# choderalab/pymbar

Measured on AMD Instinct MI355X. Metric: mbar_adaptive_iterations_per_sec, higher is better.
Workload: dtype f64

## Files before the change

### pymbar_amd/csrc/mbar_capi.cpp

```cpp
#include "mbar_ctx.h"

using namespace mbar;
using namespace mbar::host;

namespace mbar {
namespace host {

int fail(mbar_ctx* c, int code, const std::string& msg) {
    if (c) c->error = msg;
    g_last_error = msg;
    return code;
}
hipEvent_t get_event(mbar_ctx* c) {
    if (!c->pool.empty()) {
        hipEvent_t e = c->pool.back();
        c->pool.pop_back();
        return e;
    }
    hipEvent_t e;
    if (hipEventCreate(&e) != hipSuccess) return nullptr;
    return e;
}
void flush_timers(mbar_ctx* c) {
    for (auto& tp : c->pending) {
// ... 611 lines not shown
    *out = c;
    return MBAR_OK;
}

void mbar_ctx_destroy(mbar_ctx* c) {
    if (!c) return;
    (void)hipSetDevice(c->device);
    if (c->stream) (void)hipStreamSynchronize(c->stream);
    flush_timers(c);
    for (auto e : c->pool) (void)hipEventDestroy(e);
    if (c->comm && g_rccl.CommDestroy) g_rccl.CommDestroy(c->comm);
    if (c->u_alloc) (void)cache_free(c->u_alloc);
    else if (c->u) (void)cache_free(c->u);
    if (c->logden[0]) (void)cache_free(c->logden[0]);
    if (c->ad) (void)cache_free(c->ad);
    if (c->P) (void)cache_free(c->P);
    if (c->pm_vec) (void)cache_free(c->pm_vec);
    if (c->pm_ld0) (void)cache_free(c->pm_ld0);
    if (c->part_g) (void)cache_free(c->part_g);
    if (c->cwsq) (void)cache_free(c->cwsq);
    if (c->chol) (void)cache_free(c->chol);
    if (c->ad_ints) (void)cache_free(c->ad_ints);
    if (c->h_ctl) (void)cache_host_free(c->h_ctl);
    if (c->ad_graph) (void)hipGraphExecDestroy(c->ad_graph);
    if (c->dn) (void)cache_free(c->dn);
    if (c->cw) (void)cache_free(c->cw);
    if (c->lden_eff) (void)cache_free(c->lden_eff);
    if (c->small) (void)cache_free(c->small);
    if (c->part) (void)cache_free(c->part);
    if (c->scratch) (void)cache_free(c->scratch);
    if (c->red) (void)cache_free(c->red);
    if (c->hred) (void)cache_host_free(c->hred);
    if (c->lognum_part) (void)cache_free(c->lognum_part);
    if (c->f_hist) (void)cache_free(c->f_hist);
    if (c->hstage) (void)cache_host_free(c->hstage);
    if (c->vec_tmp) (void)cache_free(c->vec_tmp);
    if (c->boot_idx) (void)cache_free(c->boot_idx);
    if (c->stamps) (void)hipFree(c->stamps);
    if (c->sci_graph) (void)hipGraphExecDestroy(c->sci_graph);
    if (c->stream) {
        std::lock_guard<std::mutex> lock(g_dev_mu);
        auto& pool = g_stream_pool[c->device];
        if (pool.size() < 8)
            pool.push_back(c->stream);
        else
            (void)hipStreamDestroy(c->stream);
// ... 208 lines not shown
    if (!c->vec_tmp) HIPCHK(c, cache_malloc((void**)&c->vec_tmp, (size_t)c->ld * sizeof(double)));
    int* dlabel = nullptr;
    HIPCHK(c, cache_malloc((void**)&dlabel, (size_t)c->N * sizeof(int)));
    c->vec_holds_logshift = false;
    hipError_t e = hipMemcpyAsync(c->vec_tmp, v_host, (size_t)c->N * sizeof(double), hipMemcpyHostToDevice, c->stream);
    if (e == hipSuccess) e = hipMemcpyAsync(dlabel, label_host, (size_t)c->N * sizeof(int), hipMemcpyHostToDevice, c->stream);
    if (e == hipSuccess) e = launch_fill_masked_rows(c->stream, c->u + row0 * c->ld, c->ld, c->N, nrows, c->vec_tmp, dlabel);
    if (e == hipSuccess) e = hipStreamSynchronize(c->stream);
    (void)cache_free(dlabel);
    if (e != hipSuccess) return fail(c, MBAR_ERR_HIP, std::string("mbar_ctx_fill_masked_rows: ") + hipGetErrorString(e));
    c->u_checked = false;
    c->P_valid = false;
    c->last_psum.clear();
    flush_timers(c);
    return MBAR_OK;
}

int mbar_ctx_download_u(mbar_ctx* c, double* out, int64_t ld_out) {
    if (!c || !out || ld_out < c->N) return fail(c, MBAR_ERR_ARG, "bad argument");
    HIPCHK(c, hipSetDevice(c->device));
    const double* src = c->u;
    if (c->opt_debug_download_p) {
        if (!c->P || !c->P_valid) return fail(c, MBAR_ERR_STATE, "no resident probability matrix on this context");
        src = c->P;
    }
    HIPCHK(c, hipMemcpy2DAsync(out, (size_t)ld_out * sizeof(double), src, (size_t)c->ld * sizeof(double),
                               (size_t)c->N * sizeof(double), (size_t)c->K, hipMemcpyDeviceToHost, c->stream));
    return sync_stream(c);
}

int mbar_ctx_generate_harmonic(mbar_ctx* c, uint64_t seed, const double* O_k, const double* K_k,
                               const int64_t* N_k_global, int64_t n_global0) {
    if (!c || !O_k || !K_k || !N_k_global) return fail(c, MBAR_ERR_ARG, "NULL argument");
    HIPCHK(c, hipSetDevice(c->device));
    std::vector<int64_t> cum((size_t)c->K + 1, 0);
    for (int64_t k = 0; k < c->K; ++k) cum[k + 1] = cum[k] + N_k_global[k];
    if (n_global0 < 0 || n_global0 + c->N > cum[c->K]) return fail(c, MBAR_ERR_ARG, "shard exceeds sum(N_k)");
    double* dO = d_misc(c);
    double* dK = d_misc(c) + c->Kp;
    int64_t* dC = reinterpret_cast<int64_t*>(d_misc(c) + 2 * c->Kp);
    HIPCHK(c, hipMemcpyAsync(dO, O_k, c->K * sizeof(double), hipMemcpyHostToDevice, c->stream));
    HIPCHK(c, hipMemcpyAsync(dK, K_k, c->K * sizeof(double), hipMemcpyHostToDevice, c->stream));
    HIPCHK(c, hipMemcpyAsync(dC, cum.data(), (c->K + 1) * sizeof(int64_t), hipMemcpyHostToDevice, c->stream));
    {
        ScopedTimer t(c, MBAR_TIMER_OTHER);
        HIPCHK(c, launch_generate_harmonic(c->stream, c->u, c->ld, c->N, c->K, seed, dO, dK, dC, n_global0));
    }
// ... 706 lines not shown
```

### pymbar_amd/csrc/mbar_ctx.h

```cpp
#pragma once
#include "../../include/mbar_hip.h"
#include "mbar_internal.h"

#include <dlfcn.h>
#include <sched.h>
#include <unistd.h>
#include <rccl/rccl.h>

#include <algorithm>
#include <chrono>
#include <condition_variable>
#include <cmath>
#include <cstdio>
#include <cstdlib>
#include <cstring>
#include <functional>
#include <limits>
#include <map>
#include <memory>
#include <mutex>
#include <string>
#include <atomic>
#include <thread>
#include <unordered_map>
// ... 229 lines not shown
    double* scratch = nullptr;
    size_t scratch_doubles = 0;
    double* red = nullptr;
    size_t red_doubles = 0;
    double* hred = nullptr;
    double* hstage = nullptr;
    double* lognum_part = nullptr;
    size_t lognum_part_doubles = 0;
    double* f_hist = nullptr;
    double* vec_tmp = nullptr;
    int64_t* boot_idx = nullptr;
    size_t boot_idx_words = 0;
    uint64_t boot_layout_digest[2] = {0, 0};
    int64_t boot_states = 0, boot_total = 0;
    bool boot_has_order = false;
    bool vec_holds_logshift = false;
    hipGraphExec_t sci_graph = nullptr;
    int64_t sci_graph_batch = 0, sci_graph_sig = 0;
    double sci_graph_tol = 0.0;
    double* ad = nullptr;
    int64_t ad_hist_cap = 0;
    int* ad_ints = nullptr;
    int* h_ctl = nullptr;
    hipGraphExec_t ad_graph = nullptr;
    int64_t ad_graph_batch = 0, ad_graph_sig = 0;
    double* P = nullptr;
    bool P_failed = false;
    double* pm_vec = nullptr;
    double* pm_ld0 = nullptr;
    double* part_g = nullptr;
    size_t part_g_doubles = 0;
    double* cwsq = nullptr;
    double* chol = nullptr;
    long long* stamps = nullptr;
    std::vector<double> last_psum;
    bool P_valid = false;
    std::vector<double> P_a0;
    int64_t opt_grid = 0, opt_force_generic = 0, opt_check_finite = 1, opt_sci_batch = 16, opt_timing = 0, opt_graph = 1, opt_small = 1, opt_wide = 1;
    int64_t opt_device_loop = 1, opt_adapt_batch = 8, opt_pmode = 1, opt_fused = 1, opt_quad = 1, opt_device_loop_wide = 1, opt_pcache = 1, opt_merge_select = 1, opt_sci_merged = 1, opt_wide_pmode = 1, opt_quad_trim = 1, opt_light_last = 1, opt_direct_results = 1, opt_debug_download_p = 0, opt_fused_general = 0;
    int64_t opt_small_balanced = 1, opt_sci_pingpong = 1, opt_host_pmode = 2, opt_rect_waves = 8, opt_newton_ldlt = 1;

    ncclComm_t comm = nullptr;
    mbar_loopback* loop = nullptr;
    mbar_allreduce_fn host_reduce = nullptr;
    void* host_reduce_user = nullptr;
    int rank = 0, nranks = 1;
// ... 220 lines not shown
```

### pymbar_amd/csrc/mbar_internal.h

```cpp
#pragma once
#include <hip/hip_runtime.h>
#include <stdint.h>

#include "../../include/mbar_hip.h"

namespace mbar {

constexpr int TS = 16;
constexpr int GROUPS = 4;
constexpr int MAX_FAST_K = 256;
constexpr int PANEL = 64;

inline int64_t padded_K(int64_t K) {
    if (K <= 128) return (K + 15) / 16 * 16;
    return (K + PANEL - 1) / PANEL * PANEL;
}
inline int lse_nb_for(int64_t Kp) {
    static const int nbs[] = {1, 2, 3, 4, 5, 6, 7, 8, 12, 16};
    int need = (int)(Kp / 16);
    for (int nb : nbs) if (nb >= need) return nb;
    return 0;
}

#if defined(__HIPCC__)
// ... 164 lines not shown
    int64_t hist_cap;
    int pmode;
    const double* a0;
    double* ccur;
    int fused;
    double* cgram;
    int light_ok;
    long long* stamps;
    int newton_ldlt;
};
LaunchGeom psweep_geometry(int nb, int num_cu, int64_t ntiles, int64_t grid_override);
hipError_t launch_psweep(hipStream_t s, int nb, int nf, const LaunchGeom& g, const double* P, int64_t ld, int64_t N,
                         const double* cmul, const double* cw, double* rinv0, double* rinv1, double* psum_part,
                         const LoopCtl& lc = LoopCtl());
LaunchGeom fused_geometry(int nb, int num_cu, int64_t ntiles, int64_t grid_override, bool unit = false);
hipError_t launch_fused(hipStream_t s, int nb, const LaunchGeom& g, const double* P, int64_t ld, int64_t N, const double* cmul,
                        const double* cw, const double* wsq, bool unit, double* rinv_base, double* gram_part, double* psum_part,
                        const LoopCtl& lc);
LaunchGeom build_sweep_geometry(int nb, int num_cu, int64_t ntiles, int64_t grid_override);
hipError_t launch_build_sweep(hipStream_t s, int nb, const LaunchGeom& g, const double* u, int64_t ld, int64_t N,
                              const double* aden, const double* cw, double* P, double* rinv_slot, double* psum_part);
LaunchGeom build_gram_geometry(int nb, int num_cu, int64_t ntiles, int64_t grid_override);
hipError_t launch_build_gram(hipStream_t s, int nb, const LaunchGeom& g, const double* u, int64_t ld, int64_t N,
                             const double* aden, const double* wsq, bool general, double* P, double* rinv_slot, double* gram_part);

hipError_t launch_make_p(hipStream_t s, int num_cu, const double* u, int64_t ld, int64_t N, int64_t rows, const double* aden,
                         const double* logden, double* P);
hipError_t launch_fill(hipStream_t s, double* v, double value, int64_t n);
hipError_t launch_zero(hipStream_t s, void* p, size_t bytes);
hipError_t launch_sqrt_vec(hipStream_t s, double* dst, const double* src, int64_t n);
hipError_t launch_rinv_from_logden(hipStream_t s, const double* ld0, const double* ldv, const double* cw, bool weighted, int64_t N,
                                   double* out);
hipError_t launch_rinv_weighted(hipStream_t s, const double* rinv, const double* cw, int64_t N, double* out,
                                const LoopCtl& lc = LoopCtl());
hipError_t launch_newton(hipStream_t s, const AdaptArgs& a);
constexpr size_t NEWTON_CHOL_WORK = (size_t)256 * 256 + 8;
hipError_t launch_newton_chol(hipStream_t s, const AdaptArgs& a, double* work);
hipError_t launch_select(hipStream_t s, const AdaptArgs& a);
hipError_t launch_select_newton(hipStream_t s, const AdaptArgs& a);
hipError_t launch_ctl_resume(hipStream_t s, int* ctl);


enum : int { KDE_GAUSSIAN = 0, KDE_TOPHAT = 1, KDE_EPANECHNIKOV = 2, KDE_EXPONENTIAL = 3, KDE_LINEAR = 4, KDE_COSINE = 5 };
constexpr int KDE_MAX_D = 8;
constexpr int KDE_TILE = 64;
constexpr int KDE_MAX_CB = 32;
struct KdeLaunch {
    int kernel, d, cb;
    const double* X;
    int64_t ldx;
    const double* V;
    const double* Q;
    int64_t ldq, M;
    double coef;
    double h, inv_h, inv_h2;
    int64_t qblocks, nchunks, chunk;
    double* part;
};
size_t kde_lds_bytes(int kernel, int d, int cb);
hipError_t launch_kde(hipStream_t s, const KdeLaunch& a);
hipError_t launch_kde_combine(hipStream_t s, const KdeLaunch& a, int cv, const double* logW, double lognorm, double* out, int* flag);
hipError_t launch_kde_exact(hipStream_t s, const KdeLaunch& a, int64_t N, int64_t npairs, const int64_t* pq, const double* logW,
                            double lognorm, double* out);
// ... 418 lines not shown
```

### pymbar_amd/csrc/mbar_k_pmode.hip

```cpp
#include "mbar_device.h"

namespace mbar {

__global__ void __launch_bounds__(256)
k_rinv_weighted(const double* __restrict__ rinv, const double* __restrict__ cw, int64_t N, double* __restrict__ out,
                const int* __restrict__ ctl, int64_t slot_stride) {
    if (ctl) {
        if (ctl[CTL_DONE] != 0) return;
        rinv += (int64_t)ctl[CTL_SLOT] * slot_stride;
    }
    for (int64_t n = (int64_t)blockIdx.x * blockDim.x + threadIdx.x; n < N; n += (int64_t)gridDim.x * blockDim.x)
        out[n] = rinv[n] * sqrt(cw[n]);
}

__global__ void __launch_bounds__(256)
k_rinv_from_logden(const double* __restrict__ ld0, const double* __restrict__ ldv, const double* __restrict__ cw, int weighted,
                   int64_t N, double* __restrict__ out) {
    for (int64_t n = (int64_t)blockIdx.x * blockDim.x + threadIdx.x; n < N; n += (int64_t)gridDim.x * blockDim.x) {
        double r = exp(ld0[n] - ldv[n]);
        if (weighted) r *= sqrt(cw[n]);
        out[n] = r;
    }
}
hipError_t launch_rinv_from_logden(hipStream_t s, const double* ld0, const double* ldv, const double* cw, bool weighted, int64_t N,
// ... 502 lines not shown
    return stage_offsets_wide(ld) ? go(k_build_sweep<NB, true>) : go(k_build_sweep<NB, false>);
}
LaunchGeom build_sweep_geometry(int nb, int num_cu, int64_t ntiles, int64_t grid_override) {
    return lse_geometry(nb, 1, num_cu, ntiles, grid_override, 1);
}
hipError_t launch_build_sweep(hipStream_t s, int nb, const LaunchGeom& g, const double* u, int64_t ld, int64_t N,
                              const double* aden, const double* cw, double* P, double* rinv_slot, double* pp) {
    switch (nb) {
#define MBAR_CASE(NB_) \
    case NB_: return launch_build_sweep_nb<NB_>(s, g, u, ld, N, aden, cw, P, rinv_slot, pp);
        MBAR_CASE(1) MBAR_CASE(2) MBAR_CASE(3) MBAR_CASE(4) MBAR_CASE(5) MBAR_CASE(6) MBAR_CASE(7) MBAR_CASE(8)
#undef MBAR_CASE
        default: return hipErrorInvalidValue;
    }
}

LaunchGeom build_gram_geometry(int nb, int num_cu, int64_t ntiles, int64_t grid_override) {
    LaunchGeom g = fused_geometry(nb, num_cu, ntiles, grid_override);
    g.lds_bytes = (size_t)4 * 2 * ((size_t)nb * 16 * TS * 8 + TS * 8) + EXP_TABLE_BYTES;
    return g;
}
template <int NB>
static hipError_t launch_build_gram_nb(hipStream_t s, const LaunchGeom& g, const double* u, int64_t ld, int64_t N,
                                       const double* aden, const double* wsq, bool general, double* P, double* rinv_slot, double* gp) {
    auto go = [&](auto kern) -> hipError_t {
        if (g.lds_bytes > 64 * 1024) {
            hipError_t e = hipFuncSetAttribute(reinterpret_cast<const void*>(kern),
                                               hipFuncAttributeMaxDynamicSharedMemorySize, (int)g.lds_bytes);
            if (e != hipSuccess) return e;
        }
        const int64_t ntiles = (N + TS - 1) / TS;
        hipLaunchKernelGGL(kern, dim3(g.blocks), dim3(256), g.lds_bytes, s, u, ld, N, ntiles, aden, wsq, P, rinv_slot, gp);
        return hipGetLastError();
    };
    if (general) return stage_offsets_wide(ld) ? go(k_build_gram<NB, true, true>) : go(k_build_gram<NB, false, true>);
    return stage_offsets_wide(ld) ? go(k_build_gram<NB, true, false>) : go(k_build_gram<NB, false, false>);
}
hipError_t launch_build_gram(hipStream_t s, int nb, const LaunchGeom& g, const double* u, int64_t ld, int64_t N,
                             const double* aden, const double* wsq, bool general, double* P, double* rinv_slot, double* gram_part) {
    switch (nb) {
#define MBAR_CASE(NB_) \
    case NB_: return launch_build_gram_nb<NB_>(s, g, u, ld, N, aden, wsq, general, P, rinv_slot, gram_part);
        MBAR_CASE(1) MBAR_CASE(2) MBAR_CASE(3) MBAR_CASE(4) MBAR_CASE(5) MBAR_CASE(6) MBAR_CASE(7) MBAR_CASE(8)
#undef MBAR_CASE
        default: return hipErrorInvalidValue;
    }
}

}
```

### pymbar_amd/csrc/mbar_k_solver.hip

```cpp
#include "mbar_device.h"

namespace mbar {

__global__ void __launch_bounds__(256)
k_reduce(const double* __restrict__ part, int64_t nparts, int64_t count, int64_t chunk,
         double* __restrict__ out) {
    const int64_t i = (int64_t)blockIdx.x * blockDim.x + threadIdx.x;
    if (i >= count) return;
    const int64_t p0 = (int64_t)blockIdx.y * chunk;
    const int64_t p1 = p0 + chunk < nparts ? p0 + chunk : nparts;
    double s = 0.0;
#pragma unroll 8
    for (int64_t p = p0; p < p1; ++p) s += part[p * count + i];
    out[(int64_t)blockIdx.y * count + i] = s;
}

constexpr int LN_ROWS = 8;
constexpr int LN_TILE = 64;
template <bool MASKED>
__device__ __forceinline__ void lognum_tile(const double* __restrict__ u, int64_t ld, int64_t N, int64_t K, int64_t k0,
                                            int64_t n, const double* __restrict__ logden, const double (&a)[LN_ROWS],
                                            double (&m)[LN_ROWS], double (&s)[LN_ROWS]) {
    const bool ok = !MASKED || n < N;
    const int64_t nn = ok ? n : 0;
// ... 1188 lines not shown
    select_body(q, gram_in_lds ? select_dyn_lds : nullptr, st);
    __syncthreads();
    if (st && threadIdx.x == 0) st[1] = clock64();
    newton_body_ldlt<NB>(q, select_dyn_lds, gram_in_lds ? select_dyn_lds : nullptr, st);
    if (st && threadIdx.x == 0) st[5] = clock64();
}

__global__ void __launch_bounds__(256)
k_loop_reduce(LoopSrc src, int64_t count, int op, double* __restrict__ out) {
    const int64_t i = (int64_t)blockIdx.x * blockDim.x + threadIdx.x;
    if (i >= count) return;
    double v = src.p[0][i];
    for (int r = 1; r < src.n; ++r) v = op == 0 ? v + src.p[r][i] : fmax(v, src.p[r][i]);
    out[i] = v;
}

__global__ void k_ctl_resume(int* ctl) {
    if (threadIdx.x == 0 && ctl[CTL_DONE] == 3) {
        ctl[CTL_DONE] = 0;
        ctl[CTL_NEEDGRAM] = 0;
    }
}



hipError_t launch_reduce(hipStream_t s, const double* part, int64_t nparts, int64_t count, double* scratch,
                         double* out) {
    const unsigned gx = (unsigned)((count + 255) / 256);
    if (nparts <= 32) {
        hipLaunchKernelGGL(k_reduce, dim3(gx, 1), dim3(256), 0, s, part, nparts, count, nparts, out);
        return hipGetLastError();
    }
    const int64_t chunk = 32;
    const int64_t n1 = (nparts + chunk - 1) / chunk;
    hipLaunchKernelGGL(k_reduce, dim3(gx, (unsigned)n1), dim3(256), 0, s, part, nparts, count, chunk, scratch);
    hipLaunchKernelGGL(k_reduce, dim3(gx, 1), dim3(256), 0, s, (const double*)scratch, n1, count, n1, out);
    return hipGetLastError();
}

static int64_t lognum_tiles_per_chunk(int64_t N, int64_t K) {
    const int64_t ntiles = (N + LN_TILE - 1) / LN_TILE;
    const int64_t nsb = (K + LN_ROWS - 1) / LN_ROWS;
    int64_t target = 16384 / nsb;
    if (target < 1) target = 1;
    int64_t tpc = (ntiles + target - 1) / target;
    return tpc < 1 ? 1 : tpc;
// ... 237 lines not shown
    if (count < 1 || src.n < 1 || src.n > 8) return hipErrorInvalidValue;
    hipLaunchKernelGGL(k_loop_reduce, dim3((unsigned)((count + 255) / 256)), dim3(256), 0, s, src, count, op, out);
    return hipGetLastError();
}

hipError_t launch_newton_chol(hipStream_t s, const AdaptArgs& a, double* work) {
    const int M = a.m - 1;
    if (M < 0 || M > CHOL_NP - 1 || a.Kp > 256) return hipErrorInvalidValue;
    double* Aw = work;
    double* thr = work + (size_t)CHOL_NP * CHOL_NP;
    hipLaunchKernelGGL(k_chol_setup, dim3(CHOL_NP / 16, CHOL_NP / 16), dim3(256), 0, s, a, Aw, thr);
    for (int j0 = 0; j0 < M; j0 += CB) {
        hipLaunchKernelGGL(k_chol_panel, dim3(1), dim3(256), 0, s, a, Aw, (const double*)thr, j0);
        const int rows_below = M + 1 - (j0 + CB);
        if (rows_below > 0) {
            const int nt = (rows_below + CB - 1) / CB;
            hipLaunchKernelGGL(k_chol_update, dim3((unsigned)(nt * (nt + 1) / 2)), dim3(256), 0, s, a, Aw, j0);
        }
    }
    hipLaunchKernelGGL(k_chol_finish, dim3(1), dim3(256), 0, s, a, (const double*)Aw);
    return hipGetLastError();
}

hipError_t launch_ctl_resume(hipStream_t s, int* ctl) {
    hipLaunchKernelGGL(k_ctl_resume, dim3(1), dim3(64), 0, s, ctl);
    return hipGetLastError();
}

hipError_t launch_select_newton(hipStream_t s, const AdaptArgs& a) {
    const int M = a.m - 1;
    if (M > 127 || a.Kp > 128) return hipErrorInvalidValue;
    const int stage = (a.fused && a.Kp == 128) ? 1 : 0;
    const size_t lds = a.newton_ldlt ? (size_t)LDLT_LDS_DOUBLES * sizeof(double) : stage ? (size_t)SELECT_GRAM_LDS_DOUBLES * sizeof(double) : 0;
    auto go = [&](auto kern) -> hipError_t {
        if (lds > 48 * 1024) {
            hipError_t e = hipFuncSetAttribute(reinterpret_cast<const void*>(kern), hipFuncAttributeMaxDynamicSharedMemorySize, (int)lds);
            if (e != hipSuccess) return e;
        }
        hipLaunchKernelGGL(kern, dim3(1), dim3(256), lds, s, a, stage);
        return hipGetLastError();
    };
    if (a.newton_ldlt) return a.Kp <= 64 ? go(k_select_newton_ldlt<4>) : go(k_select_newton_ldlt<8>);
    if (M <= 63) return go(k_select_newton<4>);
    return go(k_select_newton<8>);
}

// ... 81 lines not shown
```

### pymbar_amd/csrc/mbar_loops.cpp

```cpp
#include "mbar_ctx.h"

using namespace mbar;
using namespace mbar::host;

namespace mbar {
namespace host {

int adaptive_host_loop(mbar_ctx* c, std::vector<double>& f, double tol, int64_t maxiter, int64_t min_sc_iter, double gamma,
                       int check_convergence, double* history, int64_t history_rows, mbar_solve_result& res,
                       std::vector<double>& psum, double& max_delta) {
    const int64_t K = c->K;
    const int m = (int)c->sampled.size();
    const int first = c->sampled[0];
    std::vector<double> f_old(K), cand(2 * (size_t)K), psum2(2 * (size_t)K);
    std::vector<double> H((size_t)m * m), g(m), x;
    std::vector<int> pos((size_t)K, -1);
    for (int i = 0; i < m; ++i) pos[(size_t)c->sampled[i]] = i;
    psum.assign(K, 0.0);
    int cur = 0;
    int rc = eval_core(c, f.data(), 1, 0, c->logden[cur], nullptr, psum.data(), nullptr, nullptr);
    if (rc) return rc;
    bool done = false;
    const GramPlan plan = plan_for(c);
    const bool dbg = std::getenv("MBAR_DEBUG_TIMING") != nullptr;
// ... 225 lines not shown
    const int64_t nit = res.iterations - it0;
    if (dbg && nit > 0)
        std::fprintf(stderr, "[mbar] adaptive (host loop): %lld it, per it: passA %.3f ms (of it unpacking %.3f), host solve %.3f ms (of it the factorisation + substitutions %.3f), passB %.3f ms, total %.3f ms\n",
                     (long long)nit, tA / nit, tA_unpack / nit, tH / nit, tH_solve / nit, tB / nit, (now_ms() - t0) / nit);
    return MBAR_OK;
}

bool device_loop_eligible(const mbar_ctx* c) {
    if (!c->opt_device_loop || !use_fast(c)) return false;
    if (c->nranks > 1 && !stream_transport(c)) return false;
    const int64_t ntiles = (c->N + TS - 1) / TS;
    const LaunchGeom gl = lse_geometry((int)(c->Kp / 16), 2, c->num_cu, ntiles, c->opt_grid, lse_variant_for(c));
    if (c->Kp > 128) return c->opt_device_loop_wide && use_quad(c) && gl.variant == 5;
    return gl.variant == 1;
}

inline size_t ad_off_f(const mbar_ctx*) { return 0; }
inline size_t ad_off_psum(const mbar_ctx* c) { return (size_t)c->Kp; }
inline size_t ad_off_cand(const mbar_ctx* c) { return (size_t)2 * c->Kp; }
inline size_t ad_off_ratio(const mbar_ctx* c) { return (size_t)4 * c->Kp; }
inline size_t ad_off_prm(const mbar_ctx* c) { return (size_t)5 * c->Kp; }
inline size_t ad_off_state(const mbar_ctx* c) { return (size_t)5 * c->Kp + 4; }
inline size_t ad_off_hist(const mbar_ctx* c) { return (size_t)5 * c->Kp + 8; }

int ensure_ad(mbar_ctx* c, int64_t hist_rows) {
    const int64_t cap = std::max<int64_t>(1024, std::min<int64_t>(hist_rows, 1 << 20));
    if (!c->ad || c->ad_hist_cap < cap) {
        int rc = drop_graphs(c);
        if (rc) return rc;
        if (c->ad) HIPCHK(c, cache_free(c->ad));
        c->ad = nullptr;
        HIPCHK(c, cache_malloc((void**)&c->ad, (ad_off_hist(c) + (size_t)4 * cap) * sizeof(double)));
        c->ad_hist_cap = cap;
    }
    if (!c->ad_ints) HIPCHK(c, cache_malloc((void**)&c->ad_ints, (size_t)(CTL_WORDS + c->Kp) * sizeof(int)));
    if (!c->h_ctl) HIPCHK(c, cache_host_malloc((void**)&c->h_ctl, (size_t)CTL_WORDS * sizeof(int)));
    return MBAR_OK;
}

int agree_all_ok(mbar_ctx* c, bool& ok) {
    if (c->nranks <= 1) return MBAR_OK;
    double v = ok ? 0.0 : 1.0;
    int rc = allreduce_host(c, &v, 1, 1);
    if (rc) return rc;
    ok = !(v > 0.0);
    return MBAR_OK;
}

int adaptive_device_loop(mbar_ctx* c, std::vector<double>& f, double tol, int64_t maxiter, int64_t min_sc_iter, double gamma,
                         int check_convergence, double* history, int64_t history_rows, mbar_solve_result& res,
                         std::vector<double>& psum, double& max_delta, bool& handed_back) {
    const int64_t K = c->K, Kp = c->Kp;
    const int m = (int)c->sampled.size();
    const int nb = (int)(Kp / 16);
    const int64_t ntiles = (c->N + TS - 1) / TS;
    handed_back = false;
    c->ld0_valid = false;
    psum.assign(K, 0.0);
    const bool wide = Kp > 128;
// ... 74 lines not shown
        if (!ok) return fail(c, MBAR_ERR_STATE, "a peer rank could not allocate its solver buffers");
        c->error = local_err;
    }
    int rc = MBAR_OK;
    LoopCtl lc_slot, lc_flat;
    lc_slot.ctl = lc_flat.ctl = c->ad_ints;
    lc_slot.slot_stride = c->ld;
    lc_slot.unclamped = lc_flat.unclamped = c->u_checked && !c->u_posinf;
    lc_slot.pmode = lc_flat.pmode = pmode;
    std::vector<double> an0((size_t)Kp), cm0((size_t)Kp, 0.0);
    build_aden(c, f.data(), an0.data(), Kp);
    bool warm = fused && c->opt_pcache && c->P_valid && (int64_t)c->P_a0.size() == Kp;
    for (int64_t k = 0; warm && k < Kp; ++k) {
        const bool live = !std::isinf(an0[k]), was = !std::isinf(c->P_a0[k]);
        if (live != was) warm = false;
        else if (live) {
            const double d = an0[k] - c->P_a0[k];
            if (!(std::fabs(d) < 200.0)) warm = false;
            cm0[k] = std::exp(d);
        }
    }
    rc = agree_all_ok(c, warm);
    if (rc) return rc;
    if (!pmode) {
        rc = eval_core(c, f.data(), 1, 0, c->logden[0], nullptr, psum.data(), nullptr, nullptr);
        if (rc) return rc;
    } else if (warm) {
        std::vector<int> z((size_t)CTL_WORDS, 0);
        HIPCHK(c, hipMemcpyAsync(c->ad_ints, z.data(), z.size() * sizeof(int), hipMemcpyHostToDevice, c->stream));
        std::copy(cm0.begin(), cm0.end(), c->hstage);
        std::copy(cm0.begin(), cm0.end(), c->hstage + Kp);
        HIPCHK(c, hipMemcpyAsync(d_aden(c), c->hstage, (size_t)2 * Kp * sizeof(double), hipMemcpyHostToDevice, c->stream));
        HIPCHK(c, hipMemsetAsync(c->red, 0, off_gram * sizeof(double), c->stream));
        {
            ScopedTimer t(c, MBAR_TIMER_OTHER);
            HIPCHK(c, launch_fused(c->stream, nb, gl, c->P, c->ld, c->N, d_aden(c), c->cw, c->weighted ? c->cwsq : c->cw, unit,
                                   c->logden[0], c->part_g, c->part, lc_slot));
        }
        HIPCHK(c, launch_reduce2(c->stream, c->part, (int64_t)rec_l, c->part_g, (int64_t)rec_g, gl.nwaves, c->scratch, c->red,
                                 c->red + off_gram));
        rc = allreduce_dev(c, c->red, (int64_t)(off_gram + rec_g), 0);
        if (rc) return rc;
        HIPCHK(c, hipMemcpyAsync(c->hred, c->red, (size_t)Kp * sizeof(double), hipMemcpyDeviceToHost, c->stream));
        rc = sync_stream(c);
        if (rc) return rc;
        for (int64_t k = 0; k < K; ++k) psum[k] = c->hred[k] * cm0[k];
// ... 17 lines not shown
        if (fused && c->weighted) {
            const double* lden = c->logden[0];
            if (c->weighted) {
                HIPCHK(c, launch_rinv_weighted(c->stream, c->logden[0], c->cw, c->N, c->lden_eff));
                lden = c->lden_eff;
            }
            LoopCtl lp;
            lp.pmode = true;
            {
                ScopedTimer t(c, MBAR_TIMER_GRAM);
                HIPCHK(c, launch_gram_quad(c->stream, nb, gg, c->P, c->ld, c->N, d_anum(c), lden, c->part_g, lp));
            }
            HIPCHK(c, launch_reduce(c->stream, c->part_g, gg.nwaves, (int64_t)rec_g, c->scratch, c->red + off_gram));
            rc = allreduce_dev(c, c->red + off_gram, (int64_t)rec_g, 0);
            if (rc) return rc;
        }
        rc = sync_stream(c);
        if (rc) return rc;
        c->P_a0 = an0;
        c->P_valid = true;
        res.builds += 1;
    } else {
        c->P_valid = false;
        build_aden(c, f.data(), c->hstage, Kp);
        HIPCHK(c, hipMemcpyAsync(d_aden(c), c->hstage, (size_t)Kp * sizeof(double), hipMemcpyHostToDevice, c->stream));
        HIPCHK(c, hipMemsetAsync(c->red, 0, off_gram * sizeof(double), c->stream));
        {
            ScopedTimer t(c, MBAR_TIMER_OTHER);
            if (fused)
                HIPCHK(c, launch_build_gram(c->stream, nb, gb, c->u, c->ld, c->N, d_aden(c), c->weighted ? c->cwsq : c->cw,
                                            c->weighted || !lc_slot.unclamped, c->P, c->logden[0], c->part_g));
            else
                HIPCHK(c, launch_build_sweep(c->stream, nb, gb, c->u, c->ld, c->N, d_aden(c), c->cw, c->P, c->logden[0], c->part));
        }
        if (fused) {
            HIPCHK(c, launch_reduce(c->stream, c->part_g, gb.nwaves, (int64_t)rec_g, c->scratch, c->red + off_gram));
            rc = allreduce_dev(c, c->red + off_gram, (int64_t)rec_g, 0);
            if (rc) return rc;
            HIPCHK(c, hipMemcpyAsync(c->hred + off_gram, c->red + off_gram, rec_g * sizeof(double), hipMemcpyDeviceToHost, c->stream));
            rc = sync_stream(c);
            if (rc) return rc;
            gram_row_sums(c->hred + off_gram, (int)nb, K, psum.data());
        } else {
            HIPCHK(c, launch_reduce(c->stream, c->part, gb.nwaves, Kp, c->scratch, c->red));
            rc = allreduce_dev(c, c->red, Kp, 0);
            if (rc) return rc;
            HIPCHK(c, hipMemcpyAsync(c->hred, c->red, (size_t)Kp * sizeof(double), hipMemcpyDeviceToHost, c->stream));
            rc = sync_stream(c);
            if (rc) return rc;
            for (int64_t k = 0; k < K; ++k) psum[k] = c->hred[k];
        }
        c->P_a0 = an0;
        c->P_valid = true;
        res.builds += 1;
    }
    double* gram_part = fused ? c->part_g : c->part;

    {
        std::vector<double> h(ad_off_hist(c), 0.0);
        for (int64_t k = 0; k < K; ++k) {
            h[ad_off_f(c) + k] = f[k];
            h[ad_off_psum(c) + k] = psum[k];
        }
        h[ad_off_prm(c) + 0] = gamma;
        h[ad_off_prm(c) + 1] = tol;
        h[ad_off_prm(c) + 2] = (double)std::min<int64_t>(min_sc_iter, 1 << 30);
        h[ad_off_prm(c) + 3] = check_convergence ? 1.0 : 0.0;
        h[ad_off_state(c)] = std::numeric_limits<double>::quiet_NaN();
        std::vector<int> hi((size_t)CTL_WORDS + Kp, 0);
        hi[CTL_NEEDGRAM] = fused ? 0 : 1;
        hi[CTL_GRAMSWEEPS] = 0;
        hi[CTL_SPEC] = 1;
        hi[CTL_SLOT] = warm ? 1 : 0;
        hi[CTL_ITER] = (int)res.iterations;
        hi[CTL_SCI] = (int)res.sci_iter;
        hi[CTL_NR] = (int)res.nr_iter;
        for (int i = 0; i < m; ++i) hi[CTL_WORDS + i] = c->sampled[i];
        std::vector<double> an((size_t)Kp);
        build_aden(c, f.data(), an.data(), Kp);
        HIPCHK(c, hipMemcpyAsync(c->ad, h.data(), h.size() * sizeof(double), hipMemcpyHostToDevice, c->stream));
        HIPCHK(c, hipMemcpyAsync(c->ad_ints, hi.data(), hi.size() * sizeof(int), hipMemcpyHostToDevice, c->stream));
        HIPCHK(c, hipMemcpyAsync(d_anum(c), an.data(), an.size() * sizeof(double), hipMemcpyHostToDevice, c->stream));
        if (pmode) {
            std::vector<double> pv((size_t)3 * Kp, 1.0);
            std::copy(c->P_a0.begin(), c->P_a0.end(), pv.begin());
            for (int64_t k = 0; k < Kp; ++k) {
                if (warm) pv[(size_t)Kp + k] = pv[(size_t)2 * Kp + k] = cm0[k];
                if (!(k < K && c->Nk[k] > 0.0)) pv[(size_t)Kp + k] = pv[(size_t)2 * Kp + k] = 0.0;
            }
            HIPCHK(c, hipMemcpyAsync(c->pm_vec, pv.data(), pv.size() * sizeof(double), hipMemcpyHostToDevice, c->stream));
        }
        HIPCHK(c, hipStreamSynchronize(c->stream));
    }
    AdaptArgs q;
    q.gram_red = c->red + off_gram;
    q.lse_red = c->red;
    q.f = c->ad + ad_off_f(c);
    q.psum = c->ad + ad_off_psum(c);
    q.cand = c->ad + ad_off_cand(c);
    q.ratio = c->ad + ad_off_ratio(c);
    q.aden = d_aden(c);
    q.anum = d_anum(c);
    q.Nk = d_Nk(c);
    q.lnNk = d_lnNk(c);
    q.sampled = c->ad_ints + CTL_WORDS;
    q.m = m;
    q.K = (int)K;
    q.Kp = (int)Kp;
    q.ctl = c->ad_ints;
    q.prm = c->ad + ad_off_prm(c);
    q.state = c->ad + ad_off_state(c);
    q.hist = c->ad + ad_off_hist(c);
    q.hist_cap = c->ad_hist_cap;
    q.pmode = pmode ? 1 : 0;
    q.a0 = c->pm_vec;
// ... 5 lines not shown
    if (const char* e = std::getenv("MBAR_NEWTON_LDLT")) q.newton_ldlt = std::atoi(e) != 0 ? 1 : 0;
    q.stamps = nullptr;
    if (std::getenv("MBAR_DEBUG_STAMPS")) {
        if (!c->stamps) HIPCHK(c, hipMalloc((void**)&c->stamps, 65 * 16 * sizeof(long long)));
        HIPCHK(c, hipMemsetAsync(c->stamps, 0, 65 * 16 * sizeof(long long), c->stream));
        q.stamps = c->stamps;
    }

    auto enqueue_gram = [&](bool timed) -> int {
        const double* lden = c->logden[0];
        LoopCtl lca = lc_slot;
        if (fused) HIPCHK(c, launch_ctl_resume(c->stream, c->ad_ints));
        if (c->weighted) {
            if (pmode)
                HIPCHK(c, launch_rinv_weighted(c->stream, c->logden[0], c->cw, c->N, c->lden_eff, lc_slot));
            else
                HIPCHK(c, launch_shift_logden(c->stream, c->logden[0], c->cw, 0.5, c->N, c->lden_eff, lc_slot));
            lden = c->lden_eff;
            lca = lc_flat;
        }
        {
            TimerPair tp{nullptr, nullptr, MBAR_TIMER_GRAM};
            if (timed) { tp.a = get_event(c); tp.b = get_event(c); }
            const bool ext = tp.a && tp.b && c->opt_timing == 2;
            if (ext) { lca.ev_start = tp.a; lca.ev_stop = tp.b; }
            if (tp.a && tp.b && !ext) (void)hipEventRecord(tp.a, c->stream);
            if (wide)
                HIPCHK(c, launch_gram_quad(c->stream, nb, gg, pmode ? c->P : c->u, c->ld, c->N, d_anum(c), lden, gram_part, lca));
            else
                HIPCHK(c, launch_gram_diag(c->stream, nb, gg, pmode ? c->P : c->u, c->ld, c->N, d_anum(c), lden, 0, gram_part,
                                           nullptr, lca));
            if (tp.a && tp.b && !ext) (void)hipEventRecord(tp.b, c->stream);
            if (tp.a && tp.b) c->pending.push_back(tp);
        }
        HIPCHK(c, launch_reduce(c->stream, gram_part, gg.nwaves, (int64_t)rec_g, c->scratch, c->red + off_gram));
        if (stream_transport(c)) {
            int r2 = allreduce_dev(c, c->red + off_gram, (int64_t)rec_g, 0);
            if (r2) return r2;
        }
        return MBAR_OK;
    };
    const bool merged = fused && !wide && c->opt_merge_select;
    bool need_newton = true;
    struct Section {
        mbar_ctx* c;
        TimerPair tp;
        Section(mbar_ctx* c_, bool on, int which) : c(c_) {
// ... 10 lines not shown
                c->pending.push_back(tp);
            }
        }
    };
    auto enqueue_iteration = [&](bool timed) -> int {
        const bool split = timed && c->opt_timing == 3;
        if (!fused) {
            int r2 = enqueue_gram(timed);
            if (r2) return r2;
        }
        {
            Section sec(c, split && (wide || !merged || need_newton), MBAR_TIMER_NEWTON);
            if (wide)
                HIPCHK(c, launch_newton_chol(c->stream, q, c->chol));
            else if (!merged || need_newton)
                HIPCHK(c, launch_newton(c->stream, q));
        }
        need_newton = false;
        double* psum_part = c->part;
        double* obj_part = c->part + (size_t)gl.nwaves * rec_l;
        {
            TimerPair tp{nullptr, nullptr, fused ? MBAR_TIMER_FUSED : MBAR_TIMER_LSE};
            if (timed) { tp.a = get_event(c); tp.b = get_event(c); }
            const bool ext = tp.a && tp.b && c->opt_timing == 2;
            LoopCtl lcb = lc_slot;
            if (ext) { lcb.ev_start = tp.a; lcb.ev_stop = tp.b; }
            if (tp.a && tp.b && !ext) (void)hipEventRecord(tp.a, c->stream);
            if (fused) {
                HIPCHK(c, launch_fused(c->stream, nb, gl, c->P, c->ld, c->N, d_aden(c), c->cw, c->weighted ? c->cwsq : c->cw, unit,
                                       c->logden[0], gram_part, psum_part, lcb));
                if (light && !wide) {
                    LoopCtl lcl = lc_slot;
                    lcl.light_only = true;
                    HIPCHK(c, launch_psweep(c->stream, nb, 2, gp, c->P, c->ld, c->N, d_aden(c), c->cw, c->logden[0], nullptr, psum_part, lcl));
                }
            } else if (pmode)
                HIPCHK(c, launch_psweep(c->stream, nb, 2, gl, c->P, c->ld, c->N, d_aden(c), c->cw, c->logden[0], nullptr, psum_part,
                                        lcb));
            else
                HIPCHK(c, launch_lse(c->stream, nb, 2, gl, c->u, c->ld, c->N, d_aden(c), c->cw, c->logden[0], nullptr,
                                     nullptr, psum_part, obj_part, lcb));
            if (tp.a && tp.b && !ext) (void)hipEventRecord(tp.b, c->stream);
            if (tp.a && tp.b) c->pending.push_back(tp);
        }
        int64_t ar_count = (int64_t)(rec_l + 2);
        {
            Section sec(c, split, MBAR_TIMER_REDUCE);
// ... 115 lines not shown
        const int64_t row1 = history ? std::min<int64_t>(std::min<int64_t>(it, history_rows), c->ad_hist_cap) : 0;
        if (row1 > it_start)
            HIPCHK(c, hipMemcpyAsync(history + 4 * it_start, c->ad + ad_off_hist(c) + 4 * it_start, (size_t)(row1 - it_start) * 4 * sizeof(double),
                                     hipMemcpyDeviceToHost, c->stream));
        HIPCHK(c, hipStreamSynchronize(c->stream));
        for (int64_t k = 0; k < K; ++k) {
            f[k] = h[ad_off_f(c) + k];
            psum[k] = h[ad_off_psum(c) + k];
        }
        if (it > res.iterations) max_delta = h[ad_off_state(c)];
    }
    if (q.stamps) {
        std::vector<long long> st(65 * 16);
        HIPCHK(c, hipMemcpy(st.data(), c->stamps, st.size() * sizeof(long long), hipMemcpyDeviceToHost));
        for (int i = 0; i < 64; ++i) {
            const long long* p = st.data() + 16 * i;
            if (!p[0] || !p[5]) continue;
            std::fprintf(stderr, "[mbar] k_select_newton launch %d (shader clocks): select %lld, set-up %lld, elimination %lld, solution %lld, candidates %lld, total %lld; of the elimination: pivot loops %lld, exchange + trailing update %lld; of the selection: inputs %lld, Gram staged %lld, matrix-vector product %lld, sums %lld, maxima %lld\n",
                         i, p[1] - p[0], p[2] - p[1], p[3] - p[2], p[4] - p[3], p[5] - p[4], p[5] - p[0], p[6], p[7], p[8] - p[0], p[9] - p[8], p[10] - p[9],
                         p[11] - p[10], p[12] - p[11]);
        }
    }
    res.iterations = it;
    res.sci_iter = c->h_ctl[CTL_SCI];
    res.nr_iter = c->h_ctl[CTL_NR];
    res.gram_sweeps += fused ? gram_sweeps : (int32_t)(it - it_start);
    res.light_sweeps += c->h_ctl[CTL_LIGHTS];
    if (fused && !wide && unit) res.fused_unit += 1;
    if (handed_back) {
        c->P_valid = false;
        static const char* why[] = {"", "the Newton system is not positive definite", "a candidate is too far from the point the sweeps are anchored at",
                                    "a candidate is not finite"};
        const int r = c->h_ctl[CTL_REASON];
        c->error = std::string("device-resident adaptive loop handed back to the host loop: ") + why[(r >= 1 && r <= 3) ? r : 0];
    }
    return MBAR_OK;
}


}
}

extern "C" {

int mbar_solve_adaptive(mbar_ctx* c, double* f_inout, double tol, int64_t maxiter, int64_t min_sc_iter, double gamma,
                        int check_convergence, double* history, int64_t history_rows, mbar_solve_result* result) {
    if (c && c->ext_base) return fail(c, MBAR_ERR_STATE, "mbar_solve_adaptive: an extension context holds rows only (mbar_lognum_ext / mbar_gram_w_ext sweep them)");
    if (!c || !f_inout) return fail(c, MBAR_ERR_ARG, "NULL argument");
    if (!c->have_Nk) return fail(c, MBAR_ERR_STATE, "mbar_ctx_set_Nk has not been called");
    HIPCHK(c, hipSetDevice(c->device));
    const double t0 = now_ms();
    const int64_t K = c->K;
    std::vector<double> f(f_inout, f_inout + K), psum;
    mbar_solve_result res;
    std::memset(&res, 0, sizeof(res));
    struct Ld0Guard {
        mbar_ctx* c;
        ~Ld0Guard() { c->ld0_valid = false; }
    } ld0_guard{c};
    c->ld0_valid = false;
    double max_delta = std::numeric_limits<double>::quiet_NaN();
    int rc = refresh_poison(c);
    if (rc) return rc;
    bool on_device = device_loop_eligible(c) && !c->u_poison && f_is_finite(c, f.data(), 1) && maxiter > 0;
    int handbacks = 0;
    while (on_device) {
        bool handed_back = false;
        rc = adaptive_device_loop(c, f, tol, maxiter, min_sc_iter, gamma, check_convergence, history, history_rows, res, psum,
                                  max_delta, handed_back);
        if (rc) return rc;
        if (!handed_back) break;
        const int reason = c->h_ctl[CTL_REASON];
        const bool one_off = (reason == 2 || reason == 3) && ++handbacks <= 6 && res.iterations + 1 < maxiter;
        if (!one_off) {
            on_device = false;
            break;
        }
        rc = adaptive_host_loop(c, f, tol, res.iterations + 1, min_sc_iter, gamma, check_convergence, history, history_rows, res,
                                psum, max_delta);
        if (rc) return rc;
        if (res.success || !f_is_finite(c, f.data(), 1)) break;
    }
    if (!on_device && !res.success && res.iterations < maxiter) {
        rc = adaptive_host_loop(c, f, tol, maxiter, min_sc_iter, gamma, check_convergence, history, history_rows, res, psum,
                                max_delta);
        if (rc) return rc;
    }
// ... 272 lines not shown
```

Before: 284.0.

## Stage adaptive-loop state in one pinned upload and compute gram row sums on device

```diff
diff --git a/pymbar_amd/csrc/mbar_capi.cpp b/pymbar_amd/csrc/mbar_capi.cpp
--- a/pymbar_amd/csrc/mbar_capi.cpp
+++ b/pymbar_amd/csrc/mbar_capi.cpp
@@ -657,6 +657,8 @@
     if (c->chol) (void)cache_free(c->chol);
     if (c->ad_ints) (void)cache_free(c->ad_ints);
     if (c->h_ctl) (void)cache_host_free(c->h_ctl);
+    if (c->ad_stage) (void)cache_free(c->ad_stage);
+    if (c->h_ad_stage) (void)cache_host_free(c->h_ad_stage);
     if (c->ad_graph) (void)hipGraphExecDestroy(c->ad_graph);
     if (c->dn) (void)cache_free(c->dn);
     if (c->cw) (void)cache_free(c->cw);
@@ -911,7 +913,7 @@
     const double* src = c->u;
     if (c->opt_debug_download_p) {
         if (!c->P || !c->P_valid) return fail(c, MBAR_ERR_STATE, "no resident probability matrix on this context");
-        src = c->P;
+        src = c->opt_debug_download_p == 2 ? c->P + (c->ld - c->N) : c->P;
     }
     HIPCHK(c, hipMemcpy2DAsync(out, (size_t)ld_out * sizeof(double), src, (size_t)c->ld * sizeof(double),
                                (size_t)c->N * sizeof(double), (size_t)c->K, hipMemcpyDeviceToHost, c->stream));
diff --git a/pymbar_amd/csrc/mbar_ctx.h b/pymbar_amd/csrc/mbar_ctx.h
--- a/pymbar_amd/csrc/mbar_ctx.h
+++ b/pymbar_amd/csrc/mbar_ctx.h
@@ -275,6 +275,8 @@
     int64_t ad_hist_cap = 0;
     int* ad_ints = nullptr;
     int* h_ctl = nullptr;
+    double* ad_stage = nullptr;
+    double* h_ad_stage = nullptr;
     hipGraphExec_t ad_graph = nullptr;
     int64_t ad_graph_batch = 0, ad_graph_sig = 0;
     double* P = nullptr;
diff --git a/pymbar_amd/csrc/mbar_internal.h b/pymbar_amd/csrc/mbar_internal.h
--- a/pymbar_amd/csrc/mbar_internal.h
+++ b/pymbar_amd/csrc/mbar_internal.h
@@ -210,7 +210,8 @@
                               const double* aden, const double* cw, double* P, double* rinv_slot, double* psum_part);
 LaunchGeom build_gram_geometry(int nb, int num_cu, int64_t ntiles, int64_t grid_override);
 hipError_t launch_build_gram(hipStream_t s, int nb, const LaunchGeom& g, const double* u, int64_t ld, int64_t N,
-                             const double* aden, const double* wsq, bool general, double* P, double* rinv_slot, double* gram_part);
+                             const double* aden, const double* wsq, bool general, double* P, double* rinv_slot, double* gram_part,
+                             hipEvent_t ev_start = nullptr, hipEvent_t ev_stop = nullptr);
 
 hipError_t launch_make_p(hipStream_t s, int num_cu, const double* u, int64_t ld, int64_t N, int64_t rows, const double* aden,
                          const double* logden, double* P);
@@ -227,6 +228,14 @@
 hipError_t launch_select(hipStream_t s, const AdaptArgs& a);
 hipError_t launch_select_newton(hipStream_t s, const AdaptArgs& a);
 hipError_t launch_ctl_resume(hipStream_t s, int* ctl);
+hipError_t launch_gram_row_sums(hipStream_t s, const double* blocks, int nb, int K, double* psum);
+struct StateUnpack {
+    const double* src;
+    double *ad, *anum, *aden, *pm_vec, *zero;
+    int* ints;
+    int n_ad, n_vec, n_pm, n_ints, n_zero;
+};
+hipError_t launch_unpack_state(hipStream_t s, const StateUnpack& a);
 
 
 enum : int { KDE_GAUSSIAN = 0, KDE_TOPHAT = 1, KDE_EPANECHNIKOV = 2, KDE_EXPONENTIAL = 3, KDE_LINEAR = 4, KDE_COSINE = 5 };
diff --git a/pymbar_amd/csrc/mbar_k_pmode.hip b/pymbar_amd/csrc/mbar_k_pmode.hip
--- a/pymbar_amd/csrc/mbar_k_pmode.hip
+++ b/pymbar_amd/csrc/mbar_k_pmode.hip
@@ -548,7 +548,8 @@
 }
 template <int NB>
 static hipError_t launch_build_gram_nb(hipStream_t s, const LaunchGeom& g, const double* u, int64_t ld, int64_t N,
-                                       const double* aden, const double* wsq, bool general, double* P, double* rinv_slot, double* gp) {
+                                       const double* aden, const double* wsq, bool general, double* P, double* rinv_slot, double* gp,
+                                       hipEvent_t ev_start, hipEvent_t ev_stop) {
     auto go = [&](auto kern) -> hipError_t {
         if (g.lds_bytes > 64 * 1024) {
             hipError_t e = hipFuncSetAttribute(reinterpret_cast<const void*>(kern),
@@ -556,17 +557,22 @@
             if (e != hipSuccess) return e;
         }
         const int64_t ntiles = (N + TS - 1) / TS;
-        hipLaunchKernelGGL(kern, dim3(g.blocks), dim3(256), g.lds_bytes, s, u, ld, N, ntiles, aden, wsq, P, rinv_slot, gp);
+        if (ev_start && ev_stop)
+            hipExtLaunchKernelGGL(kern, dim3(g.blocks), dim3(256), g.lds_bytes, s, ev_start, ev_stop, 0, u, ld, N, ntiles, aden, wsq, P,
+                                  rinv_slot, gp);
+        else
+            hipLaunchKernelGGL(kern, dim3(g.blocks), dim3(256), g.lds_bytes, s, u, ld, N, ntiles, aden, wsq, P, rinv_slot, gp);
         return hipGetLastError();
     };
     if (general) return stage_offsets_wide(ld) ? go(k_build_gram<NB, true, true>) : go(k_build_gram<NB, false, true>);
     return stage_offsets_wide(ld) ? go(k_build_gram<NB, true, false>) : go(k_build_gram<NB, false, false>);
 }
 hipError_t launch_build_gram(hipStream_t s, int nb, const LaunchGeom& g, const double* u, int64_t ld, int64_t N,
-                             const double* aden, const double* wsq, bool general, double* P, double* rinv_slot, double* gram_part) {
+                             const double* aden, const double* wsq, bool general, double* P, double* rinv_slot, double* gram_part,
+                             hipEvent_t ev_start, hipEvent_t ev_stop) {
     switch (nb) {
 #define MBAR_CASE(NB_) \
-    case NB_: return launch_build_gram_nb<NB_>(s, g, u, ld, N, aden, wsq, general, P, rinv_slot, gram_part);
+    case NB_: return launch_build_gram_nb<NB_>(s, g, u, ld, N, aden, wsq, general, P, rinv_slot, gram_part, ev_start, ev_stop);
         MBAR_CASE(1) MBAR_CASE(2) MBAR_CASE(3) MBAR_CASE(4) MBAR_CASE(5) MBAR_CASE(6) MBAR_CASE(7) MBAR_CASE(8)
 #undef MBAR_CASE
         default: return hipErrorInvalidValue;
diff --git a/pymbar_amd/csrc/mbar_k_solver.hip b/pymbar_amd/csrc/mbar_k_solver.hip
--- a/pymbar_amd/csrc/mbar_k_solver.hip
+++ b/pymbar_amd/csrc/mbar_k_solver.hip
@@ -1234,6 +1234,44 @@
     }
 }
 
+__global__ void __launch_bounds__(128) k_gram_row_sums(const double* __restrict__ blocks, int nb, int K, double* __restrict__ psum) {
+    const int k = blockIdx.x * blockDim.x + threadIdx.x;
+    if (k >= K) return;
+    const int A = k >> 4, a = k & 15;
+    auto blk = [&](int I, int J) { return blocks + (size_t)(I * nb - I * (I - 1) / 2 + (J - I)) * 256; };
+    double acc = 0.0;
+    for (int I = 0; I < A; ++I) {
+        const double* b = blk(I, A);
+        for (int r = 0; r < 16; ++r) acc = __dadd_rn(acc, b[r * 16 + a]);
+    }
+    {
+        const double* b = blk(A, A);
+        for (int r = 0; r < a; ++r) acc = __dadd_rn(acc, b[r * 16 + a]);
+        for (int q = a; q < 16; ++q) acc = __dadd_rn(acc, b[a * 16 + q]);
+    }
+    for (int J = A + 1; J < nb; ++J) {
+        const double* b = blk(A, J);
+        for (int q = 0; q < 16; ++q) acc = __dadd_rn(acc, b[a * 16 + q]);
+    }
+    psum[k] = acc;
+}
+
+__global__ void __launch_bounds__(256) k_unpack_state(StateUnpack a) {
+    const int i = blockIdx.x * blockDim.x + threadIdx.x;
+    const double* src = a.src;
+    if (i < a.n_ad) a.ad[i] = src[i];
+    src += a.n_ad;
+    if (i < a.n_vec) {
+        a.anum[i] = src[i];
+        if (a.aden) a.aden[i] = src[i];
+    }
+    src += a.n_vec;
+    if (a.pm_vec && i < a.n_pm) a.pm_vec[i] = src[i];
+    src += a.n_pm;
+    if (i < a.n_ints) a.ints[i] = reinterpret_cast<const int*>(src)[i];
+    if (i < a.n_zero) a.zero[i] = 0.0;
+}
+
 
 
 hipError_t launch_reduce(hipStream_t s, const double* part, int64_t nparts, int64_t count, double* scratch,
@@ -1517,6 +1555,15 @@
     return hipGetLastError();
 }
 
+hipError_t launch_gram_row_sums(hipStream_t s, const double* blocks, int nb, int K, double* psum) {
+    hipLaunchKernelGGL(k_gram_row_sums, dim3((K + 127) / 128), dim3(128), 0, s, blocks, nb, K, psum);
+    return hipGetLastError();
+}
+hipError_t launch_unpack_state(hipStream_t s, const StateUnpack& a) {
+    const int n = std::max(std::max(std::max(a.n_ad, a.n_vec), std::max(a.n_pm, a.n_ints)), a.n_zero);
+    hipLaunchKernelGGL(k_unpack_state, dim3((n + 255) / 256), dim3(256), 0, s, a);
+    return hipGetLastError();
+}
 hipError_t launch_ctl_resume(hipStream_t s, int* ctl) {
     hipLaunchKernelGGL(k_ctl_resume, dim3(1), dim3(64), 0, s, ctl);
     return hipGetLastError();
diff --git a/pymbar_amd/csrc/mbar_loops.cpp b/pymbar_amd/csrc/mbar_loops.cpp
--- a/pymbar_amd/csrc/mbar_loops.cpp
+++ b/pymbar_amd/csrc/mbar_loops.cpp
@@ -271,6 +271,7 @@
 inline size_t ad_off_prm(const mbar_ctx* c) { return (size_t)5 * c->Kp; }
 inline size_t ad_off_state(const mbar_ctx* c) { return (size_t)5 * c->Kp + 4; }
 inline size_t ad_off_hist(const mbar_ctx* c) { return (size_t)5 * c->Kp + 8; }
+inline size_t ad_stage_doubles(const mbar_ctx* c) { return ad_off_hist(c) + (size_t)4 * c->Kp + ((size_t)CTL_WORDS + c->Kp + 1) / 2; }
 
 int ensure_ad(mbar_ctx* c, int64_t hist_rows) {
     const int64_t cap = std::max<int64_t>(1024, std::min<int64_t>(hist_rows, 1 << 20));
@@ -284,6 +285,8 @@
     }
     if (!c->ad_ints) HIPCHK(c, cache_malloc((void**)&c->ad_ints, (size_t)(CTL_WORDS + c->Kp) * sizeof(int)));
     if (!c->h_ctl) HIPCHK(c, cache_host_malloc((void**)&c->h_ctl, (size_t)CTL_WORDS * sizeof(int)));
+    if (!c->ad_stage) HIPCHK(c, cache_malloc((void**)&c->ad_stage, ad_stage_doubles(c) * sizeof(double)));
+    if (!c->h_ad_stage) HIPCHK(c, cache_host_malloc((void**)&c->h_ad_stage, ad_stage_doubles(c) * sizeof(double)));
     return MBAR_OK;
 }
 
@@ -404,6 +407,56 @@
     }
     rc = agree_all_ok(c, warm);
     if (rc) return rc;
+    auto upload_state = [&](bool to_aden) -> int {
+        double* h = c->h_ad_stage;
+        std::fill(h, h + ad_stage_doubles(c), 0.0);
+        for (int64_t k = 0; k < K; ++k) {
+            h[ad_off_f(c) + k] = f[k];
+            h[ad_off_psum(c) + k] = psum[k];
+        }
+        h[ad_off_prm(c) + 0] = gamma;
+        h[ad_off_prm(c) + 1] = tol;
+        h[ad_off_prm(c) + 2] = (double)std::min<int64_t>(min_sc_iter, 1 << 30);
+        h[ad_off_prm(c) + 3] = check_convergence ? 1.0 : 0.0;
+        h[ad_off_state(c)] = std::numeric_limits<double>::quiet_NaN();
+        double* an = h + ad_off_hist(c);
+        std::copy(an0.begin(), an0.end(), an);
+        double* pv = an + Kp;
+        if (pmode) {
+            const std::vector<double>& a0 = warm ? c->P_a0 : an0;
+            for (int64_t k = 0; k < Kp; ++k) {
+                pv[k] = a0[k];
+                const double cm = !(k < K && c->Nk[k] > 0.0) ? 0.0 : warm ? cm0[k] : 1.0;
+                pv[(size_t)Kp + k] = pv[(size_t)2 * Kp + k] = cm;
+            }
+        }
+        int* hi = reinterpret_cast<int*>(pv + 3 * Kp);
+        hi[CTL_NEEDGRAM] = fused ? 0 : 1;
+        hi[CTL_GRAMSWEEPS] = 0;
+        hi[CTL_SPEC] = 1;
+        hi[CTL_SLOT] = warm ? 1 : 0;
+        hi[CTL_ITER] = (int)res.iterations;
+        hi[CTL_SCI] = (int)res.sci_iter;
+        hi[CTL_NR] = (int)res.nr_iter;
+        for (int i = 0; i < m; ++i) hi[CTL_WORDS + i] = c->sampled[i];
+        HIPCHK(c, hipMemcpyAsync(c->ad_stage, h, ad_stage_doubles(c) * sizeof(double), hipMemcpyHostToDevice, c->stream));
+        StateUnpack su;
+        su.src = c->ad_stage;
+        su.ad = c->ad;
+        su.anum = d_anum(c);
+        su.aden = to_aden ? d_aden(c) : nullptr;
+        su.pm_vec = pmode ? c->pm_vec : nullptr;
+        su.zero = c->red;
+        su.ints = c->ad_ints;
+        su.n_ad = (int)ad_off_hist(c);
+        su.n_vec = (int)Kp;
+        su.n_pm = (int)(3 * Kp);
+        su.n_ints = (int)(CTL_WORDS + Kp);
+        su.n_zero = to_aden ? (int)off_gram : 0;
+        HIPCHK(c, launch_unpack_state(c->stream, su));
+        return MBAR_OK;
+    };
+    bool state_up = false;
     if (!pmode) {
         rc = eval_core(c, f.data(), 1, 0, c->logden[0], nullptr, psum.data(), nullptr, nullptr);
         if (rc) return rc;
@@ -467,25 +520,29 @@
         res.builds += 1;
     } else {
         c->P_valid = false;
-        build_aden(c, f.data(), c->hstage, Kp);
-        HIPCHK(c, hipMemcpyAsync(d_aden(c), c->hstage, (size_t)Kp * sizeof(double), hipMemcpyHostToDevice, c->stream));
-        HIPCHK(c, hipMemsetAsync(c->red, 0, off_gram * sizeof(double), c->stream));
-        {
+        if (fused) {
+            rc = upload_state(true);
+            if (rc) return rc;
+            state_up = true;
+            TimerPair tp{nullptr, nullptr, MBAR_TIMER_OTHER};
+            if (c->opt_timing) { tp.a = get_event(c); tp.b = get_event(c); }
+            const bool timed = tp.a && tp.b;
+            HIPCHK(c, launch_build_gram(c->stream, nb, gb, c->u, c->ld, c->N, d_aden(c), c->weighted ? c->cwsq : c->cw,
+                                        c->weighted || !lc_slot.unclamped, c->P, c->logden[0], c->part_g, timed ? tp.a : nullptr,
+                                        timed ? tp.b : nullptr));
+            if (timed) c->pending.push_back(tp);
+        } else {
+            build_aden(c, f.data(), c->hstage, Kp);
+            HIPCHK(c, hipMemcpyAsync(d_aden(c), c->hstage, (size_t)Kp * sizeof(double), hipMemcpyHostToDevice, c->stream));
+            HIPCHK(c, hipMemsetAsync(c->red, 0, off_gram * sizeof(double), c->stream));
             ScopedTimer t(c, MBAR_TIMER_OTHER);
-            if (fused)
-                HIPCHK(c, launch_build_gram(c->stream, nb, gb, c->u, c->ld, c->N, d_aden(c), c->weighted ? c->cwsq : c->cw,
-                                            c->weighted || !lc_slot.unclamped, c->P, c->logden[0], c->part_g));
-            else
-                HIPCHK(c, launch_build_sweep(c->stream, nb, gb, c->u, c->ld, c->N, d_aden(c), c->cw, c->P, c->logden[0], c->part));
+            HIPCHK(c, launch_build_sweep(c->stream, nb, gb, c->u, c->ld, c->N, d_aden(c), c->cw, c->P, c->logden[0], c->part));
         }
         if (fused) {
             HIPCHK(c, launch_reduce(c->stream, c->part_g, gb.nwaves, (int64_t)rec_g, c->scratch, c->red + off_gram));
             rc = allreduce_dev(c, c->red + off_gram, (int64_t)rec_g, 0);
             if (rc) return rc;
-            HIPCHK(c, hipMemcpyAsync(c->hred + off_gram, c->red + off_gram, rec_g * sizeof(double), hipMemcpyDeviceToHost, c->stream));
-            rc = sync_stream(c);
-            if (rc) return rc;
-            gram_row_sums(c->hred + off_gram, (int)nb, K, psum.data());
+            HIPCHK(c, launch_gram_row_sums(c->stream, c->red + off_gram, (int)nb, (int)K, c->ad + ad_off_psum(c)));
         } else {
             HIPCHK(c, launch_reduce(c->stream, c->part, gb.nwaves, Kp, c->scratch, c->red));
             rc = allreduce_dev(c, c->red, Kp, 0);
@@ -501,41 +558,9 @@
     }
     double* gram_part = fused ? c->part_g : c->part;
 
-    {
-        std::vector<double> h(ad_off_hist(c), 0.0);
-        for (int64_t k = 0; k < K; ++k) {
-            h[ad_off_f(c) + k] = f[k];
-            h[ad_off_psum(c) + k] = psum[k];
-        }
-        h[ad_off_prm(c) + 0] = gamma;
-        h[ad_off_prm(c) + 1] = tol;
-        h[ad_off_prm(c) + 2] = (double)std::min<int64_t>(min_sc_iter, 1 << 30);
-        h[ad_off_prm(c) + 3] = check_convergence ? 1.0 : 0.0;
-        h[ad_off_state(c)] = std::numeric_limits<double>::quiet_NaN();
-        std::vector<int> hi((size_t)CTL_WORDS + Kp, 0);
-        hi[CTL_NEEDGRAM] = fused ? 0 : 1;
-        hi[CTL_GRAMSWEEPS] = 0;
-        hi[CTL_SPEC] = 1;
-        hi[CTL_SLOT] = warm ? 1 : 0;
-        hi[CTL_ITER] = (int)res.iterations;
-        hi[CTL_SCI] = (int)res.sci_iter;
-        hi[CTL_NR] = (int)res.nr_iter;
-        for (int i = 0; i < m; ++i) hi[CTL_WORDS + i] = c->sampled[i];
-        std::vector<double> an((size_t)Kp);
-        build_aden(c, f.data(), an.data(), Kp);
-        HIPCHK(c, hipMemcpyAsync(c->ad, h.data(), h.size() * sizeof(double), hipMemcpyHostToDevice, c->stream));
-        HIPCHK(c, hipMemcpyAsync(c->ad_ints, hi.data(), hi.size() * sizeof(int), hipMemcpyHostToDevice, c->stream));
-        HIPCHK(c, hipMemcpyAsync(d_anum(c), an.data(), an.size() * sizeof(double), hipMemcpyHostToDevice, c->stream));
-        if (pmode) {
-            std::vector<double> pv((size_t)3 * Kp, 1.0);
-            std::copy(c->P_a0.begin(), c->P_a0.end(), pv.begin());
-            for (int64_t k = 0; k < Kp; ++k) {
-                if (warm) pv[(size_t)Kp + k] = pv[(size_t)2 * Kp + k] = cm0[k];
-                if (!(k < K && c->Nk[k] > 0.0)) pv[(size_t)Kp + k] = pv[(size_t)2 * Kp + k] = 0.0;
-            }
-            HIPCHK(c, hipMemcpyAsync(c->pm_vec, pv.data(), pv.size() * sizeof(double), hipMemcpyHostToDevice, c->stream));
-        }
-        HIPCHK(c, hipStreamSynchronize(c->stream));
+    if (!state_up) {
+        rc = upload_state(false);
+        if (rc) return rc;
     }
     AdaptArgs q;
     q.gram_red = c->red + off_gram;
@@ -587,7 +612,7 @@
         {
             TimerPair tp{nullptr, nullptr, MBAR_TIMER_GRAM};
             if (timed) { tp.a = get_event(c); tp.b = get_event(c); }
-            const bool ext = tp.a && tp.b && c->opt_timing == 2;
+            const bool ext = tp.a && tp.b && (c->opt_timing == 1 || c->opt_timing == 2);
             if (ext) { lca.ev_start = tp.a; lca.ev_stop = tp.b; }
             if (tp.a && tp.b && !ext) (void)hipEventRecord(tp.a, c->stream);
             if (wide)
@@ -644,7 +669,7 @@
         {
             TimerPair tp{nullptr, nullptr, fused ? MBAR_TIMER_FUSED : MBAR_TIMER_LSE};
             if (timed) { tp.a = get_event(c); tp.b = get_event(c); }
-            const bool ext = tp.a && tp.b && c->opt_timing == 2;
+            const bool ext = tp.a && tp.b && (c->opt_timing == 1 || c->opt_timing == 2);
             LoopCtl lcb = lc_slot;
             if (ext) { lcb.ev_start = tp.a; lcb.ev_stop = tp.b; }
             if (tp.a && tp.b && !ext) (void)hipEventRecord(tp.a, c->stream);
@@ -806,10 +831,12 @@
         }
     }
     res.iterations = it;
-    res.sci_iter = c->h_ctl[CTL_SCI];
-    res.nr_iter = c->h_ctl[CTL_NR];
+    if (nbatch > 0) {
+        res.sci_iter = c->h_ctl[CTL_SCI];
+        res.nr_iter = c->h_ctl[CTL_NR];
+        res.light_sweeps += c->h_ctl[CTL_LIGHTS];
+    }
     res.gram_sweeps += fused ? gram_sweeps : (int32_t)(it - it_start);
-    res.light_sweeps += c->h_ctl[CTL_LIGHTS];
     if (fused && !wide && unit) res.fused_unit += 1;
     if (handed_back) {
         c->P_valid = false;
@@ -846,7 +873,7 @@
     double max_delta = std::numeric_limits<double>::quiet_NaN();
     int rc = refresh_poison(c);
     if (rc) return rc;
-    bool on_device = device_loop_eligible(c) && !c->u_poison && f_is_finite(c, f.data(), 1) && maxiter > 0;
+    bool on_device = device_loop_eligible(c) && !c->u_poison && f_is_finite(c, f.data(), 1) && maxiter >= 0;
     int handbacks = 0;
     while (on_device) {
         bool handed_back = false;
```

Result: no change. 284.4 (median of 5 runs) (+0.2%).
